# MikeIvanichev/norma

Hardware: AMD Instinct MI355X
Metric: audio-sec/wall-sec (xRT) distil-large-v3 fp16 b32 (higher is better)
Workload: dtype f16

## Files before the change

norma_amd/csrc/k_gemm.hip:

```cpp
#include <stdlib.h>

#include <atomic>

#include "mfma_tile128.h"

#define BM 128
#define BN 128
#define BK 64

__device__ __forceinline__ float gelu_tanh_f(float v) { return gelu_tanh_fast(v); }

__device__ __forceinline__ const half_t *a_row_ptr(const GemmParams &p, int m) {
    if (m >= p.M) m = p.M - 1;
    int b = nh_div(m, p.a_rpb, p.a_magic), r = m - b * p.a_rpb;
    return p.A + (long)b * p.a_bstride + (long)r * p.lda;
}

template <bool SWAP>
__device__ __forceinline__ void gemm_mainloop(const GemmParams &p, char *smem, int m0, int n0, f32x4 (&acc)[4][4]) {
    tile128_mainloop<SWAP>([&](int row) { return a_row_ptr(p, m0 + row); },
                           [&](int row) { return p.W + (long)(n0 + row) * p.K; }, p.K / BK, smem, acc);
}

__device__ __forceinline__ long out_row(const GemmParams &p, int m) {
    int b = nh_div(m, p.o_rpb, p.o_magic), r = m - b * p.o_rpb;
    return (long)b * p.o_bstride + r + p.o_off;
}

__global__ __launch_bounds__(256, 2) void gemm_f16_kernel(GemmParams p) {
    __shared__ __attribute__((aligned(16))) char smem[T128_LDS];
    const int ntn = p.N / BN, ntm = (p.M + BM - 1) / BM;
    const int bid = xcd_contiguous(blockIdx.x, ntn * ntm);
    const int tm = bid / ntn, tn = bid - tm * ntn;
    const int m0 = tm * BM, n0 = tn * BN;
    const int lane = threadIdx.x & 63, w = threadIdx.x >> 6;
    const int wm = w >> 1, wn = w & 1;
    const int fr = lane & 15, fq = lane >> 4;

    f32x4 acc[4][4];
#pragma unroll
    for (int i = 0; i < 4; i++)
#pragma unroll
        for (int j = 0; j < 4; j++) acc[i][j] = (f32x4){0.f, 0.f, 0.f, 0.f};

    const int seg = (p.epi == EPI_F16 || p.epi == EPI_GELU_F16) ? n0 / p.seg_n : 0;
    const bool vt = (p.epi == EPI_F16 && seg == p.vt_seg);
    if (vt) gemm_mainloop<false>(p, smem, m0, n0, acc);
    else gemm_mainloop<true>(p, smem, m0, n0, acc);

    if (vt) {
        half_t *dst = reinterpret_cast<half_t *>(seg == 0 ? p.out[0] : seg == 1 ? p.out[1] : p.out[2]);
#pragma unroll
        for (int i = 0; i < 4; i++) {
            int n = n0 + wn * 64 + 16 * i + fr;
            float bv = p.bias ? p.bias[n] : 0.f;
            int nl = n - seg * p.seg_n, h = nl >> 6, dh = nl & 63;
#pragma unroll
            for (int j = 0; j < 4; j++) {
                int m = m0 + wm * 64 + 16 * j + 4 * fq;
                if (m >= p.M) continue;
                int b = nh_div(m, p.S, p.s_magic), s = m - b * p.S;
                half_t *row = dst + ((long)(b * p.H + h) * NH_DH + dh) * NH_SP;
                if (s + 3 < p.S && m + 3 < p.M) {
                    half4 v = {(half_t)(acc[i][j][0] + bv), (half_t)(acc[i][j][1] + bv),
                               (half_t)(acc[i][j][2] + bv), (half_t)(acc[i][j][3] + bv)};
                    *reinterpret_cast<half4 *>(row + s) = v;
                } else {
                    for (int r = 0; r < 4; r++) {
                        int mm = m + r;
                        if (mm >= p.M) break;
                        int bb = nh_div(mm, p.S, p.s_magic), ss = mm - bb * p.S;
                        dst[((long)(bb * p.H + h) * NH_DH + dh) * NH_SP + ss] = (half_t)(acc[i][j][r] + bv);
                    }
                }
            }
        }
        return;
    }
    half_t *obase = reinterpret_cast<half_t *>(seg == 0 ? p.out[0] : seg == 1 ? p.out[1] : p.out[2]);
#pragma unroll
    for (int i = 0; i < 4; i++) {
        const int n = n0 + wn * 64 + 16 * i + 4 * fq;
        f32x4 bv = {0.f, 0.f, 0.f, 0.f};
        if (p.bias) bv = *reinterpret_cast<const f32x4 *>(p.bias + n);
#pragma unroll
        for (int j = 0; j < 4; j++) {
            const int m = m0 + wm * 64 + 16 * j + fr;
            if (m >= p.M) continue;
            f32x4 v = acc[i][j] + bv;
            if (p.epi == EPI_F16 || p.epi == EPI_GELU_F16) {
                if (p.epi == EPI_F16 && seg == 0 && p.seg0_scale != 0.f) v *= p.seg0_scale;
                if (p.epi == EPI_GELU_F16) {
                    v[0] = gelu_tanh_f(v[0]); v[1] = gelu_tanh_f(v[1]);
                    v[2] = gelu_tanh_f(v[2]); v[3] = gelu_tanh_f(v[3]);
                }
                const int nl = n - seg * p.seg_n;
                half_t *dst = p.head_major ? obase + (((long)nh_div(m, p.S, p.s_magic) * p.H + (nl >> 6)) * p.S + (m - nh_div(m, p.S, p.s_magic) * p.S)) * NH_DH + (nl & 63)
                                           : obase + out_row(p, m) * p.ldo + nl;
                half4 hv = {(half_t)v[0], (half_t)v[1], (half_t)v[2], (half_t)v[3]};
                *reinterpret_cast<half4 *>(dst) = hv;
            } else if (p.epi == EPI_RESID_F32) {
                float *dst = reinterpret_cast<float *>(p.out[0]) + (long)m * p.ldo + n;
                f32x4 x = *reinterpret_cast<const f32x4 *>(dst);
                *reinterpret_cast<f32x4 *>(dst) = x + v;
            } else {
                int s = m - nh_div(m, p.S, p.s_magic) * p.S;
                f32x4 pe = *reinterpret_cast<const f32x4 *>(p.pos + (long)s * p.N + n);
                f32x4 o = {gelu_tanh_f(v[0]) + pe[0], gelu_tanh_f(v[1]) + pe[1], gelu_tanh_f(v[2]) + pe[2],
                           gelu_tanh_f(v[3]) + pe[3]};
                *reinterpret_cast<f32x4 *>(reinterpret_cast<float *>(p.out[0]) + (long)m * p.ldo + n) = o;
            }
        }
    }
}

#define G2_BM 256
#define G2_BN 256
#define G2_GM 4
#define PP_BUF 65536
#define PP_HT 16384
#define PP_RING (2 * PP_BUF)
#define PP_EPI_PITCH 136
#define PP_EPI_WAVE (16 * PP_EPI_PITCH)

struct PPSource { unsigned ag[2][2], wg[2][2]; };

__device__ __forceinline__ PPSource pp_source(const GemmParams &p, int m0, int n0) {
    int tid = threadIdx.x;
    asm volatile("" : "+v"(tid));
    const int lrow = tid >> 3;
    const int csrc = ((tid & 7) ^ ((lrow >> 1) & 7)) * 8;
    PPSource sg;
#pragma unroll
    for (int h = 0; h < 2; h++)
#pragma unroll
        for (int i = 0; i < 2; i++) {
            sg.ag[h][i] = (unsigned)(a_row_ptr(p, m0 + i * 128 + h * 64 + lrow) - p.A) + csrc;
            const int l = lrow + 64 * i;
            sg.wg[h][i] = (unsigned)(n0 + (l >> 5) * 64 + h * 32 + (l & 31)) * (unsigned)p.K + csrc;
        }
    return sg;
}

__device__ __forceinline__ void pp_stage(const GemmParams &p, char *wbase, const PPSource &sg, int t, int which) {
    const int h = (which >> 1) & 1;
    const bool isB = which == 1 || which == 2;
    char *dst = wbase + (t & 1) * PP_BUF + (isB ? 2 * PP_HT : 0) + h * PP_HT;
    const unsigned ko = (unsigned)t * 64u;
    if (isB) {
        __builtin_amdgcn_global_load_lds((gbl_void *)(p.W + (size_t)(sg.wg[h][0] + ko)), (lds_void *)dst, 16, 0, 0);
        __builtin_amdgcn_global_load_lds((gbl_void *)(p.W + (size_t)(sg.wg[h][1] + ko)), (lds_void *)(dst + 8192), 16, 0, 0);
    } else {
        __builtin_amdgcn_global_load_lds((gbl_void *)(p.A + (size_t)(sg.ag[h][0] + ko)), (lds_void *)dst, 16, 0, 0);
        __builtin_amdgcn_global_load_lds((gbl_void *)(p.A + (size_t)(sg.ag[h][1] + ko)), (lds_void *)(dst + 8192), 16, 0, 0);
    }
}

__device__ __forceinline__ void pp_prologue(const GemmParams &p, char *wbase, const PPSource &sg) {
    pp_stage(p, wbase, sg, 0, 0); pp_stage(p, wbase, sg, 0, 1); pp_stage(p, wbase, sg, 0, 2); pp_stage(p, wbase, sg, 0, 3);
    pp_stage(p, wbase, sg, 1, 0); pp_stage(p, wbase, sg, 1, 1);
}

template <bool SWAP>
__device__ __forceinline__ void pp_main(const GemmParams &p, char *smem, char *wbase, const PPSource &sg, f32x4 (&acc)[8][4]) {
    const int lane = threadIdx.x & 63, w = threadIdx.x >> 6;
    const int wr = w >> 2, wc = w & 3;
    const int fr = lane & 15, fq = lane >> 4;
    const int nt = p.K >> 6;
    const int offA0 = (wr * 64 + fr) * 128 + ((fq ^ (fr >> 1)) << 4);
    const int offB0 = (wc * 32 + fr) * 128 + ((fq ^ (fr >> 1)) << 4);
    const char *const pa[2] = {smem + offA0, smem + (offA0 ^ 64)};
    const char *const pb[2] = {smem + offB0, smem + (offB0 ^ 64)};
    half8 fa[4][2], fb[4][2];

#define PP_PHASE(Q, BUF, WAIT, DO_ISSUE, ST)                                                                             \
    {                                                                                                                    \
        constexpr int tb_ = (BUF) * PP_BUF;                                                                              \
        if ((Q) == 0) {                                                                                                  \
            _Pragma("unroll") for (int j = 0; j < 2; j++) _Pragma("unroll") for (int ks = 0; ks < 2; ks++)             \
                fb[j][ks] = *reinterpret_cast<const half8 *>(pb[ks] + (tb_ + 2 * PP_HT + 2048 * j));                    \
            __builtin_amdgcn_sched_barrier(0);                                                                           \
            _Pragma("unroll") for (int i = 0; i < 4; i++) _Pragma("unroll") for (int ks = 0; ks < 2; ks++)             \
                fa[i][ks] = *reinterpret_cast<const half8 *>(pa[ks] + (tb_ + 2048 * i));                               \
        } else if ((Q) == 1) {                                                                                           \
            _Pragma("unroll") for (int j = 0; j < 2; j++) _Pragma("unroll") for (int ks = 0; ks < 2; ks++)             \
                fb[2 + j][ks] = *reinterpret_cast<const half8 *>(pb[ks] + (tb_ + 3 * PP_HT + 2048 * j));                \
        } else if ((Q) == 2) {                                                                                           \
            _Pragma("unroll") for (int i = 0; i < 4; i++) _Pragma("unroll") for (int ks = 0; ks < 2; ks++)             \
                fa[i][ks] = *reinterpret_cast<const half8 *>(pa[ks] + (tb_ + PP_HT + 2048 * i));                       \
        }                                                                                                                \
        __builtin_amdgcn_sched_barrier(0);                                                                               \
        if (DO_ISSUE) pp_stage(p, wbase, sg, (ST), (Q) == 2 ? 0 : (Q) == 3 ? 1 : (Q) == 0 ? 2 : 3);                     \
        if ((WAIT) == 8) asm volatile("s_waitcnt vmcnt(8)" ::: "memory");                                                \
        else if ((WAIT) == 4) asm volatile("s_waitcnt vmcnt(4)" ::: "memory");                                           \
        else if ((WAIT) == 2) asm volatile("s_waitcnt vmcnt(2)" ::: "memory");                                           \
        else if ((WAIT) == 0) asm volatile("s_waitcnt vmcnt(0)" ::: "memory");                                           \
        __builtin_amdgcn_s_barrier();                                                                                    \
        asm volatile("s_waitcnt lgkmcnt(0)" ::: "memory");                                                               \
        __builtin_amdgcn_sched_barrier(0);                                                                               \
        __builtin_amdgcn_s_setprio(1);                                                                                   \
        {                                                                                                                \
            constexpr int ib_ = ((Q) >= 2) ? 4 : 0, jb_ = ((Q) == 1 || (Q) == 2) ? 2 : 0;                                \
            _Pragma("unroll") for (int ks = 0; ks < 2; ks++) _Pragma("unroll") for (int i = 0; i < 4; i++)             \
                _Pragma("unroll") for (int j = 0; j < 2; j++) {                                                         \
                    if (SWAP) acc[ib_ + i][jb_ + j] = __builtin_amdgcn_mfma_f32_16x16x32_f16(fb[jb_ + j][ks], fa[i][ks], acc[ib_ + i][jb_ + j], 0, 0, 0); \
                    else acc[ib_ + i][jb_ + j] = __builtin_amdgcn_mfma_f32_16x16x32_f16(fa[i][ks], fb[jb_ + j][ks], acc[ib_ + i][jb_ + j], 0, 0, 0);      \
                }                                                                                                        \
        }                                                                                                                \
        __builtin_amdgcn_s_setprio(0);                                                                                   \
        __builtin_amdgcn_sched_barrier(0);                                                                               \
        __builtin_amdgcn_s_barrier();                                                                                    \
    }

    asm volatile("s_waitcnt vmcnt(0)" ::: "memory");
    __builtin_amdgcn_s_barrier();
    if (wr == 1) __builtin_amdgcn_s_barrier();
    int t = 0;
    for (; t + 4 <= nt; t += 2) {
        PP_PHASE(0, 0, 8, true, t + 1)
        PP_PHASE(1, 0, 8, true, t + 1)
        PP_PHASE(2, 0, -1, true, t + 2)
        PP_PHASE(3, 0, 8, true, t + 2)
        PP_PHASE(0, 1, 8, true, t + 2)
        PP_PHASE(1, 1, 8, true, t + 2)
        PP_PHASE(2, 1, -1, true, t + 3)
        PP_PHASE(3, 1, 8, true, t + 3)
    }
    PP_PHASE(0, 0, 8, true, t + 1)
    PP_PHASE(1, 0, 8, true, t + 1)
    PP_PHASE(2, 0, -1, false, 0)
    PP_PHASE(3, 0, 4, false, 0)
    PP_PHASE(0, 1, 2, false, 0)
    PP_PHASE(1, 1, 0, false, 0)
    PP_PHASE(2, 1, -1, false, 0)
    PP_PHASE(3, 1, -1, false, 0)
    if (wr == 0) __builtin_amdgcn_s_barrier();
#undef PP_PHASE
}

__device__ __forceinline__ void pp_tile(int vb, int ntn, int ntm, int &tm, int &tn) {
    grouped_tile(xcd_contiguous(vb, ntn * ntm), ntn, ntm, G2_GM, tm, tn);
}

template <int EPI>
__global__ __launch_bounds__(512) void gemm256_f16_kernel(GemmParams p) {
    __shared__ __attribute__((aligned(16))) char smem[PP_RING + 8 * PP_EPI_WAVE];
    const int ntn = p.N / G2_BN, ntm = (p.M + G2_BM - 1) / G2_BM, nwg = ntn * ntm;
    const int lane = threadIdx.x & 63, w = threadIdx.x >> 6;
    const int wm = w >> 2, wn = w & 3;
    const int fr = lane & 15, fq = lane >> 4;
    char *const wbase = smem + __builtin_amdgcn_readfirstlane(w) * 1024;
    char *const img = smem + PP_RING + w * PP_EPI_WAVE;

    int vb = blockIdx.x, tm, tn;
    pp_tile(vb, ntn, ntm, tm, tn);
    PPSource sg = pp_source(p, tm * G2_BM, tn * G2_BN);
    pp_prologue(p, wbase, sg);
    for (;;) {
        const int m0 = tm * G2_BM, n0 = tn * G2_BN;
        f32x4 acc[8][4];
#pragma unroll
        for (int i = 0; i < 8; i++)
#pragma unroll
            for (int j = 0; j < 4; j++) acc[i][j] = (f32x4){0.f, 0.f, 0.f, 0.f};
        const int seg = (EPI == EPI_F16 || EPI == EPI_GELU_F16) ? n0 / p.seg_n : 0;
        const bool vt = (EPI == EPI_F16 && seg == p.vt_seg);
        if (vt) pp_main<false>(p, smem, wbase, sg, acc);
        else pp_main<true>(p, smem, wbase, sg, acc);

        f32x4 rs[4][4];
        __amdgpu_buffer_rsrc_t xrs;
        unsigned xoff = 0;
        if (EPI == EPI_RESID_F32) {
            xrs = __builtin_amdgcn_make_buffer_rsrc(p.out[0], 0, (int)((long)p.M * p.ldo * 4), 0x00020000);
            int ln = threadIdx.x;
            asm volatile("" : "+v"(ln));
            xoff = (unsigned)(((long)(m0 + (ln >> 8) * 128 + (ln & 15)) * p.ldo + n0 + ((ln >> 6) & 3) * 64 + 4 * ((ln >> 4) & 3)) * 4);
#pragma unroll
            for (int ii = 0; ii < 4; ii++)
#pragma unroll
                for (int j = 0; j < 4; j++)
                    rs[ii][j] = __builtin_bit_cast(f32x4, __builtin_amdgcn_raw_buffer_load_b128(xrs, xoff + (unsigned)(64 * ii * p.ldo + 64 * j), 0, 0));
        }
        const int nvb = vb + gridDim.x;
        const bool more = nvb < nwg;
        if (more) {
            pp_tile(nvb, ntn, ntm, tm, tn);
            sg = pp_source(p, tm * G2_BM, tn * G2_BN);
            pp_prologue(p, wbase, sg);
        }

        if (vt) {
            half_t *dst = reinterpret_cast<half_t *>(seg == 0 ? p.out[0] : seg == 1 ? p.out[1] : p.out[2]);
#pragma unroll
            for (int j = 0; j < 4; j++) {
                const float bv = p.bias ? p.bias[n0 + wn * 64 + 16 * j + fr] : 0.f;
#pragma unroll
                for (int hh = 0; hh < 2; hh++) {
#pragma unroll
                    for (int ii = 0; ii < 4; ii++) {
                        const f32x4 a = acc[4 * hh + ii][j];
                        half4 v = {(half_t)(a[0] + bv), (half_t)(a[1] + bv), (half_t)(a[2] + bv), (half_t)(a[3] + bv)};
                        *reinterpret_cast<half4 *>(img + fr * PP_EPI_PITCH + (16 * ii + 4 * fq) * 2) = v;
                    }
#pragma unroll
                    for (int it = 0; it < 2; it++) {
                        const int nrow = 8 * it + (lane >> 3), mc = (lane & 7) * 8;
                        const half4 lo = *reinterpret_cast<const half4 *>(img + nrow * PP_EPI_PITCH + mc * 2);
                        const half4 hi = *reinterpret_cast<const half4 *>(img + nrow * PP_EPI_PITCH + mc * 2 + 8);
                        const int n = n0 + wn * 64 + 16 * j + nrow, nl = n - seg * p.seg_n, h = nl >> 6, dh = nl & 63;
                        const int m = m0 + wm * 128 + 64 * hh + mc;
                        if (m >= p.M) continue;
                        const int b = nh_div(m, p.S, p.s_magic), ss = m - b * p.S;
                        if (ss + 7 < p.S && m + 7 < p.M) {
                            half8 o = {lo[0], lo[1], lo[2], lo[3], hi[0], hi[1], hi[2], hi[3]};
                            *reinterpret_cast<half8 *>(dst + ((long)(b * p.H + h) * NH_DH + dh) * NH_SP + ss) = o;
                        } else {
                            for (int r = 0; r < 8; r++) {
                                const int mm = m + r;
                                if (mm >= p.M) break;
                                const int bb = nh_div(mm, p.S, p.s_magic), s2 = mm - bb * p.S;
                                dst[((long)(bb * p.H + h) * NH_DH + dh) * NH_SP + s2] = r < 4 ? lo[r] : hi[r - 4];
                            }
                        }
                    }
                }
            }
        } else if (EPI == EPI_F16 || EPI == EPI_GELU_F16) {
            half_t *ob = reinterpret_cast<half_t *>(seg == 0 ? p.out[0] : seg == 1 ? p.out[1] : p.out[2]);
            f32x4 bv[4];
#pragma unroll
            for (int j = 0; j < 4; j++) {
                bv[j] = (f32x4){0.f, 0.f, 0.f, 0.f};
                if (p.bias) bv[j] = *reinterpret_cast<const f32x4 *>(p.bias + n0 + wn * 64 + 16 * j + 4 * fq);
            }
            const int ncol = n0 + wn * 64 - seg * p.seg_n + (lane & 7) * 8;
            const bool q_scaled = EPI == EPI_F16 && seg == 0 && p.seg0_scale != 0.f;
#pragma unroll
            for (int i = 0; i < 8; i++) {
#pragma unroll
                for (int j = 0; j < 4; j++) {
                    f32x4 v = acc[i][j] + bv[j];
                    if (EPI == EPI_F16 && q_scaled) v *= p.seg0_scale;
                    if (EPI == EPI_GELU_F16) {
                        v[0] = gelu_tanh_f(v[0]); v[1] = gelu_tanh_f(v[1]); v[2] = gelu_tanh_f(v[2]); v[3] = gelu_tanh_f(v[3]);
                    }
                    half4 hv = {(half_t)v[0], (half_t)v[1], (half_t)v[2], (half_t)v[3]};
                    *reinterpret_cast<half4 *>(img + fr * PP_EPI_PITCH + (16 * j + 4 * fq) * 2) = hv;
                }
#pragma unroll
                for (int it = 0; it < 2; it++) {
                    const int mr = 8 * it + (lane >> 3);
                    const int m = m0 + wm * 128 + 16 * i + mr;
                    const half4 lo = *reinterpret_cast<const half4 *>(img + mr * PP_EPI_PITCH + (lane & 7) * 16);
                    const half4 hi = *reinterpret_cast<const half4 *>(img + mr * PP_EPI_PITCH + (lane & 7) * 16 + 8);
                    if (m < p.M) {
                        half8 o = {lo[0], lo[1], lo[2], lo[3], hi[0], hi[1], hi[2], hi[3]};
                        half_t *dst = p.head_major ? ob + (((long)nh_div(m, p.S, p.s_magic) * p.H + (ncol >> 6)) * p.S + (m - nh_div(m, p.S, p.s_magic) * p.S)) * NH_DH + (lane & 7) * 8
                                                   : ob + out_row(p, m) * p.ldo + ncol;
                        *reinterpret_cast<half8 *>(dst) = o;
                    }
                }
            }
        } else if (EPI == EPI_RESID_F32) {
            f32x4 bv[4];
#pragma unroll
            for (int j = 0; j < 4; j++) {
                bv[j] = (f32x4){0.f, 0.f, 0.f, 0.f};
                if (p.bias) bv[j] = *reinterpret_cast<const f32x4 *>(p.bias + n0 + wn * 64 + 16 * j + 4 * fq);
            }
#pragma unroll
            for (int ii = 0; ii < 4; ii++)
#pragma unroll
                for (int j = 0; j < 4; j++)
                    __builtin_amdgcn_raw_buffer_store_b128(__builtin_bit_cast(u32x4, rs[ii][j] + (acc[ii][j] + bv[j])), xrs, xoff + (unsigned)(64 * ii * p.ldo + 64 * j), 0, 0);
#pragma unroll
            for (int ii = 0; ii < 4; ii++)
#pragma unroll
                for (int j = 0; j < 4; j++)
                    rs[ii][j] = __builtin_bit_cast(f32x4, __builtin_amdgcn_raw_buffer_load_b128(xrs, xoff + (unsigned)(64 * (4 + ii) * p.ldo + 64 * j), 0, 0));
#pragma unroll
            for (int ii = 0; ii < 4; ii++)
#pragma unroll
                for (int j = 0; j < 4; j++)
                    __builtin_amdgcn_raw_buffer_store_b128(__builtin_bit_cast(u32x4, rs[ii][j] + (acc[4 + ii][j] + bv[j])), xrs, xoff + (unsigned)(64 * (4 + ii) * p.ldo + 64 * j), 0, 0);
        } else {
#pragma unroll
            for (int j = 0; j < 4; j++) {
                const int n = n0 + wn * 64 + 16 * j + 4 * fq;
                f32x4 bv = {0.f, 0.f, 0.f, 0.f};
                if (p.bias) bv = *reinterpret_cast<const f32x4 *>(p.bias + n);
#pragma unroll
                for (int i = 0; i < 8; i++) {
                    const int m = m0 + wm * 128 + 16 * i + fr;
                    if (m >= p.M) continue;
                    const f32x4 v = acc[i][j] + bv;
                    const int s = m - nh_div(m, p.S, p.s_magic) * p.S;
                    const f32x4 pe = *reinterpret_cast<const f32x4 *>(p.pos + (long)s * p.N + n);
                    f32x4 o = {gelu_tanh_f(v[0]) + pe[0], gelu_tanh_f(v[1]) + pe[1], gelu_tanh_f(v[2]) + pe[2],
                               gelu_tanh_f(v[3]) + pe[3]};
                    *reinterpret_cast<f32x4 *>(reinterpret_cast<float *>(p.out[0]) + (long)m * p.ldo + n) = o;
                }
            }
        }
        if (!more) break;
        vb = nvb;
    }
}

static int device_cu_count() {
    static std::atomic<int> cus[NH_MAX_DEVICES];
    int dev = 0;
    if (hipGetDevice(&dev) != hipSuccess || dev < 0 || dev >= NH_MAX_DEVICES) return 256;
    int n = cus[dev].load(std::memory_order_relaxed);
    if (!n) {
        if (hipDeviceGetAttribute(&n, hipDeviceAttributeMultiprocessorCount, dev) != hipSuccess || n <= 0) n = 256;
        cus[dev].store(n, std::memory_order_relaxed);
    }
    return n;
}

static GemmParams with_magics(const GemmParams &p_in) {
    GemmParams p = p_in;
    const long max_m = (long)p.M - 1;
    p.a_magic = nh_magic(p.a_rpb, max_m); p.o_magic = nh_magic(p.o_rpb, max_m); p.s_magic = nh_magic(p.S, max_m);
    return p;
}

void launch_gemm(const GemmParams &p_in, hipStream_t st) {
    const GemmParams p = with_magics(p_in);
    const bool seg_ok = (p.epi != EPI_F16 && p.epi != EPI_GELU_F16) || (p.seg_n % G2_BN == 0);
    if (p.N % G2_BN == 0 && p.K % 128 == 0 && seg_ok && p.M >= G2_BM) {
        const int nwg = (p.N / G2_BN) * ((p.M + G2_BM - 1) / G2_BM);
        int cus = p.cus > 0 ? p.cus : device_cu_count();
        cus -= cus % 8;
        const dim3 grid(nwg < cus ? nwg : cus), block(512);
        switch (p.epi) {
            case EPI_F16: hipLaunchKernelGGL(gemm256_f16_kernel<EPI_F16>, grid, block, 0, st, p); break;
            case EPI_GELU_F16: hipLaunchKernelGGL(gemm256_f16_kernel<EPI_GELU_F16>, grid, block, 0, st, p); break;
            case EPI_RESID_F32: hipLaunchKernelGGL(gemm256_f16_kernel<EPI_RESID_F32>, grid, block, 0, st, p); break;
            default: hipLaunchKernelGGL(gemm256_f16_kernel<EPI_CONV2_F32>, grid, block, 0, st, p); break;
        }
        return;
    }
    launch_gemm_128(p, st);
}

void launch_gemm_128(const GemmParams &p_in, hipStream_t st) {
    const GemmParams p = with_magics(p_in);
    int ntn = p.N / BN, ntm = (p.M + BM - 1) / BM;
    hipLaunchKernelGGL(gemm_f16_kernel, dim3(ntn * ntm), dim3(256), 0, st, p);
}
```

norma_amd/csrc/nh_kernels.h:

```cpp
#pragma once
#include <hip/hip_runtime.h>
#include <math.h>
#include <stdint.h>

#include <atomic>

#include "skinny_plan.h"

typedef _Float16 half_t;
typedef __attribute__((ext_vector_type(8))) _Float16 half8;
typedef __attribute__((ext_vector_type(4))) _Float16 half4;
typedef __attribute__((ext_vector_type(2))) _Float16 half2v;
typedef __attribute__((ext_vector_type(2))) float f32x2;
typedef __attribute__((ext_vector_type(4))) float f32x4;
typedef __attribute__((ext_vector_type(16))) float f32x16;
typedef __attribute__((ext_vector_type(4))) unsigned int u32x4;

#define NH_MELP 128
#define NH_SP 1536
#define NH_DH 64
#define NH_MAX_DEVICES 64
#define NH_MAX_VOCAB 65536

enum GemmEpi {
    EPI_F16 = 0,
    EPI_GELU_F16 = 1,
    EPI_RESID_F32 = 2,
    EPI_CONV2_F32 = 3,
};

struct GemmParams {
    const half_t *A; long lda; int a_rpb; long a_bstride;
    const half_t *W;
    const float *bias;
    int M, N, K;
    int epi;
    void *out[3]; int seg_n; long ldo;
    int o_rpb; long o_bstride; long o_off;
    int vt_seg;
    int head_major;
    float seg0_scale;
    int S, H;
    const float *pos;
    int cus;
    unsigned a_magic, o_magic, s_magic;
};
static inline unsigned nh_magic(int d, long max_m) {
    if (d <= 0 || (long)d > max_m) return 0u;
    if ((unsigned long long)max_m * (unsigned long long)d >= 0x100000000ull) return ~0u;
    return (unsigned)((0x100000000ull + (unsigned)d - 1) / (unsigned)d);
}
#ifdef __HIPCC__
__device__ __forceinline__ int nh_div(int m, int d, unsigned magic) {
    return magic == 0u ? 0 : magic == ~0u ? m / d : (int)__umulhi((unsigned)m, magic);
}
#endif
void launch_gemm(const GemmParams &p, hipStream_t st);
void launch_gemm_128(const GemmParams &p, hipStream_t st);

struct SkinnyParams {
    const half_t *x; long ldx;
    const half_t *W; const float *bias;
    const half_t *Wt;
    int R, N, K;
    int epi;
    void *out[3]; long ldo;
    int d, t0, Tn, ctx;
    const int32_t *pos_ptr;
    const float *ln_x, *ln_w, *ln_b;
    float ln_rk;
};
inline bool skinny_ln_supported(int R, int N, int K) { return skinny_plan(R, N, K, SK_F32, false, true).kind != SKP_NONE; }

#ifdef __HIPCC__
__device__ __forceinline__ float gelu_tanh_fast(float v) {
#pragma clang fp contract(off)
    const float k0 = -2.0f * 0.7978845608028654f * 1.4426950408889634f;
    const float k1 = k0 * 0.044715f;
    const float m = v * __builtin_fmaf(v * v, k1, k0);
    float r = v * __builtin_amdgcn_rcpf(1.0f + __builtin_amdgcn_exp2f(m));
    asm("" : "+v"(r));
    return r;
}
__device__ __forceinline__ float ln_sum8(float acc, const f32x4 &a, const f32x4 &b) {
#pragma clang fp contract(off)
    acc += (a[0] + a[1]) + (a[2] + a[3]);
    acc += (b[0] + b[1]) + (b[2] + b[3]);
    return acc;
}
__device__ __forceinline__ float ln_sq8(float acc, const f32x4 &a, const f32x4 &b, float mean) {
#pragma clang fp contract(off)
    const f32x4 t = a - mean, u = b - mean;
    acc += __builtin_fmaf(t[1], t[1], t[0] * t[0]) + __builtin_fmaf(t[3], t[3], t[2] * t[2]);
    acc += __builtin_fmaf(u[1], u[1], u[0] * u[0]) + __builtin_fmaf(u[3], u[3], u[2] * u[2]);
    return acc;
}
__device__ __forceinline__ float ln_mean(float sum, float rk) {
#pragma clang fp contract(off)
    return sum * rk;
}
__device__ __forceinline__ float ln_inv(float sumsq, float rk) {
#pragma clang fp contract(off)
    const float var = sumsq * rk;
    return 1.0f / sqrtf(var + 1e-5f);
}
__device__ __forceinline__ f32x4 ln_apply(const f32x4 &x, float mean, float inv, const f32x4 &g, const f32x4 &b) {
#pragma clang fp contract(off)
    const f32x4 t = (x - mean) * inv;
    f32x4 o = {__builtin_fmaf(t[0], g[0], b[0]), __builtin_fmaf(t[1], g[1], b[1]), __builtin_fmaf(t[2], g[2], b[2]),
               __builtin_fmaf(t[3], g[3], b[3])};
    asm("" : "+v"(o));
    return o;
}
#endif
bool launch_layernorm_sliced(const float *x, const float *w, const float *b, half_t *y, float *y32, int M, int K, hipStream_t st);
[[nodiscard]] bool launch_skinny(const SkinnyParams &p, hipStream_t st);
void launch_repack_tiles(const half_t *W, half_t *out, int N, int K, hipStream_t st);

#define NH_LDS_EXCLUSIVE (160 * 1024)
#ifdef __HIPCC__
static inline size_t lds_exclusive_bytes(size_t needed) {
#ifdef NH_DBG_SHARE_LDS
    return needed;
#else
    (void)needed;
    return (size_t)NH_LDS_EXCLUSIVE;
#endif
}
template <auto Kernel, class... Args>
static void launch_lds_exclusive(dim3 grid, dim3 block, size_t lds_used, hipStream_t st, Args... args) {
    static std::atomic<bool> attr_set[NH_MAX_DEVICES];
    int dev = 0;
    (void)hipGetDevice(&dev);
    if (dev < 0 || dev >= NH_MAX_DEVICES || !attr_set[dev].load(std::memory_order_acquire)) {
        hipFuncSetAttribute(reinterpret_cast<const void *>(Kernel), hipFuncAttributeMaxDynamicSharedMemorySize, NH_LDS_EXCLUSIVE);
        if (dev >= 0 && dev < NH_MAX_DEVICES) attr_set[dev].store(true, std::memory_order_release);
    }
    hipLaunchKernelGGL(Kernel, grid, block, lds_exclusive_bytes(lds_used), st, args...);
}
#endif

void launch_layernorm(const float *x, const float *w, const float *b, half_t *y, float *y32, int M, int d,
                      hipStream_t st);
void launch_embed(const int32_t *tokens, int tok_stride, const half_t *E, const half_t *P, float *x, int B,
                  int Tn, int t0, const int32_t *pos_ptr, int d, hipStream_t st);

#ifdef __HIPCC__
template <typename T> __device__ __forceinline__ float sample_to_f32(T v);
template <> __device__ __forceinline__ float sample_to_f32<float>(float v) { return v; }
template <> __device__ __forceinline__ float sample_to_f32<double>(double v) { return (float)v; }
template <> __device__ __forceinline__ float sample_to_f32<int8_t>(int8_t v) { return (float)v * (1.0f / 128.0f); }
template <> __device__ __forceinline__ float sample_to_f32<int16_t>(int16_t v) { return (float)v * (1.0f / 32768.0f); }
template <> __device__ __forceinline__ float sample_to_f32<int32_t>(int32_t v) { return (float)v * (1.0f / 2147483648.0f); }
template <> __device__ __forceinline__ float sample_to_f32<int64_t>(int64_t v) { return (float)v * (1.0f / 9223372036854775808.0f); }
template <> __device__ __forceinline__ float sample_to_f32<uint8_t>(uint8_t v) { return (float)((int)v - 128) * (1.0f / 128.0f); }
template <> __device__ __forceinline__ float sample_to_f32<uint16_t>(uint16_t v) { return (float)((int)v - 32768) * (1.0f / 32768.0f); }
template <> __device__ __forceinline__ float sample_to_f32<uint32_t>(uint32_t v) { return (float)(int32_t)(v ^ 0x80000000u) * (1.0f / 2147483648.0f); }
template <> __device__ __forceinline__ float sample_to_f32<uint64_t>(uint64_t v) { return (float)(int64_t)(v ^ 0x8000000000000000ull) * (1.0f / 9223372036854775808.0f); }
#endif

struct ResampleClip {
    long long off;
    long long num0;
    int n_frames;
    int n_out;
};
struct ResampleParams {
    const void *frames;
    int dtype, channels;
    const ResampleClip *clips; int batch;
    const float *coef;
    int L, M, T;
    float *out; long out_stride;
    int max_out;
};
#define NH_RS_TILE 2048
static inline size_t resample_lds_bytes(int L, int M, int T) {
    return sizeof(float) * (size_t)(((long long)(NH_RS_TILE - 1) * M + L - 1) / L + T + 2);
}
[[nodiscard]] bool launch_resample(const ResampleParams &p, hipStream_t st);

#define NH_CUT_FRAME 160
#define NH_CUT_TILE 128
#define NH_CUT_ROW 161
static inline size_t cut_lds_bytes() { return sizeof(float) * (size_t)NH_CUT_TILE * NH_CUT_ROW; }
void launch_cut_energy(const float *pcm, long long n_valid, float *e, long long n_frames, hipStream_t st);
void launch_cut_window(const float *e, float *E, long long F, int W, hipStream_t st);
struct CutSearch {
    const float *E; long long F;
    int min_frames, max_frames;
    long long n_samples;
    long long *starts; int32_t *lens;
    int32_t *count;
    long long cap;
};
void launch_cut_search(const CutSearch &p, hipStream_t st);
#ifdef __HIPCC__
__device__ __forceinline__ void cut_merge(float &best, int &c, float ob, int oc) {
    if (oc >= 0 && (c < 0 || ob < best || (ob == best && oc > c))) { best = ob; c = oc; }
}
__device__ __forceinline__ int cut_search_range(const float *E, long long s, int min_frames, int max_frames, float *w_best, int *w_c) {
    const int tid = threadIdx.x;
    float best = INFINITY;
    int c = -1;
    for (int r = min_frames + tid; r <= max_frames; r += 256) {
        const float v = E[s + r];
        if (v <= best) { best = v; c = r; }
    }
#pragma unroll
    for (int off = 32; off > 0; off >>= 1) {
        const float ob = __shfl_xor(best, off);
        const int oc = __shfl_xor(c, off);
        cut_merge(best, c, ob, oc);
    }
    if ((tid & 63) == 0) { w_best[tid >> 6] = best; w_c[tid >> 6] = c; }
    __syncthreads();
    best = w_best[0]; c = w_c[0];
    for (int w = 1; w < 4; w++) cut_merge(best, c, w_best[w], w_c[w]);
    __syncthreads();
    return c < 0 ? max_frames : c;
}
#endif

#define NH_VAD_HIST_TILE 4096
#define NH_VAD_TILE 2048
struct VadSelect {
    unsigned hist[2][256];
    unsigned prefix[2];
    long long rank[2];
    int parted;
    int n_valid;
};
struct VadLevels {
    int lo_permille, hi_permille;
    float lo_ratio, hi_ratio, abs_floor;
};
void launch_vad_hist(const float *E, long long F, int shift, VadSelect *sel, hipStream_t st);
void launch_vad_pick(VadSelect *sel, int shift, const VadLevels &lv, float *levels, hipStream_t st);
struct VadShape {
    const float *E; const float *levels;
    long long F;
    const uint8_t *in; uint8_t *out;
    const int *carry_l, *carry_r;
    int *tile_l, *tile_r;
    int min_speech, pad, min_gap;
    long long *regions; const int *carry_n;
};
void launch_vad_shape(int step, const VadShape &p, hipStream_t st);
void launch_vad_carry(const int *tile_l, const int *tile_r, int *carry_l, int *carry_r, int n_tiles, long long F, int sum, int *total, hipStream_t st);
struct VadPieces {
    const float *E; const long long *regions; const int *n_regions;
    int min_frames, max_frames;
    long long n_samples;
    long long *starts; int32_t *lens; long long cap_pieces;
    int32_t *chunk_first; long long cap_chunks;
    int32_t *counts;
};
void launch_vad_pieces(const VadPieces &p, hipStream_t st);
struct VadGather {
    const float *src; float *dst; long long dst_stride;
    const long long *tab;
    int n_pieces, vec4;
};
void launch_vad_gather(const VadGather &p, int batch, long long max_total, hipStream_t st);

struct MelTables {
    const float *hann;
    const float *dft_cos;
    const float *dft_sin;
    const float *tw_cos;
    const float *tw_sin;
    const float *filters;
};
void launch_logmel_grp(const float *pcm, const int32_t *n_samples, long stride, const MelTables &t,
                       const int32_t *grp, int n_mel, int frames, float *mel32, unsigned *chunk_max, int B,
                       hipStream_t st);
void launch_mel_finish_ex(float *mel32, const unsigned *chunk_max, half_t *img, int B, int n_mel, int frames,
                          int normalise, hipStream_t st);

#define NH_ENC_Q_SCALE (0.125f * 1.4426950408889634f)
void launch_enc_attention(const half_t *q, const half_t *k, long ld, const half_t *vt, half_t *out, long ldo,
                          int B, int S, int H, hipStream_t st);

void launch_dec_attention(const half_t *q, const half_t *kc, const half_t *vc, half_t *out, int B, int H, int d, int ctx, int Tk,
                          const int32_t *pos_ptr, hipStream_t st, const int32_t *done);

bool launch_prefill_self_attention(const half_t *q, const half_t *k, const half_t *v, long ld, half_t *out, long ldo, half_t *ck,
                                   half_t *cv, int B, int T, int H, int C, hipStream_t st);
bool launch_prefill_cross_attention(const half_t *q, long ldq, const half_t *ck, const half_t *cv, half_t *out, long ldo, int B, int T,
                                    int H, int S, hipStream_t st);

void launch_xabs_attention(const half_t *q, const half_t *Wkv, const float *bkv, const half_t *xa, half_t *U, half_t *out, int B, int H, int d, int S,
                           const int32_t *done, hipStream_t st);

bool xabs_fast_supported(int d, int H);
void launch_transpose_sq(const half_t *in, half_t *out, int d, hipStream_t st);
void launch_xabs_attention_fast(const half_t *q, const half_t *WkT, const half_t *Wkv, const float *bkv, const half_t *xa, half_t *U, float *zpart, float *mlpart,
                                half_t *out, int B, int H, int d, int S, const int32_t *done, hipStream_t st);

struct DecodeState {
    int32_t *tokens;
    int32_t *n_tokens;
    int32_t *done;
    int32_t *have_last;
    int32_t *last_ts;
    double *sum_logprob;
    double *no_speech;
    int32_t *n_active;
    const uint8_t *suppress;
};
struct RuleTokens { int sot, eot, lang, task, no_speech, no_timestamps, zero_sec, one_sec; };
inline int nh_logits_ld(int V) { return (V + 63) & ~63; }
void launch_logit_step(const float *logits, int V, DecodeState s, RuleTokens tk, int B, int ctx, int cap,
                       int max_new, int prompt_len, int mode, float *partials, unsigned *tickets, int32_t *pos_ptr,
                       hipStream_t st, const int32_t *handled = nullptr);
void launch_pool_admit(DecodeState s, int32_t *pos, unsigned *tickets, int row, int ctx, int t0, int t1, int t2, int P, hipStream_t st,
                       int32_t *detect_flag = nullptr, int detect = 0);
struct PoolSampling {
    float *inv_t;
    unsigned long long *seed;
    unsigned *clip, *attempt;
    int32_t *handled;
};
void launch_pool_retry(DecodeState s, int32_t *pos, unsigned *tickets, PoolSampling ps, int row, int P, float inv_t,
                       unsigned long long seed, unsigned clip, unsigned attempt, hipStream_t st, int32_t *detect_flag = nullptr);
void launch_pool_sample_step(const float *logits, int V, DecodeState s, RuleTokens tk, int B, int ctx, int cap, int max_new,
                             int prompt_len, PoolSampling ps, int32_t *pos, hipStream_t st);
void launch_sample_step(const float *logits, int V, DecodeState s, RuleTokens tk, int B, int ctx, int cap, int max_new,
                        int prompt_len, float inv_t, unsigned long long seed, unsigned clip0, unsigned attempt, hipStream_t st);
void launch_sample_rules(const float *probs_in, int32_t *token_out, const int32_t *tokens, int n_tokens, int last_ts,
                         const uint8_t *suppress, RuleTokens tk, int V, float inv_t, unsigned long long seed, unsigned clip,
                         unsigned attempt, hipStream_t st);
void launch_lang_detect(const float *logits, int V, const int32_t *lang_tokens, int n, float *probs_out, int32_t *lang_out,
                        int B, hipStream_t st);
struct PoolDetect {
    const int32_t *flag;
    const int32_t *lang_tokens;
    int n;
    int32_t *lang_out;
    float *probs;
};
void launch_pool_lang_detect(const float *logits, int V, DecodeState s, int B, int ctx, const int32_t *pos, PoolDetect det,
                             hipStream_t st);
#define NH_GUARD_MAX_BIAS 256
#define NH_GUARD_MAX_PERIOD 64
#define NH_GUARD_MAX_HISTORY 512
struct GuardSpec { int ngram; float penalty; int loop_period, loop_repeats, bias; };
struct GuardBufs {
    const int32_t *bias_tok;
    const float *bias_val;
    const int32_t *bias_n;
    const int32_t *bias_map;
    int bias_mod;
    int32_t *loop_exit;
};
void launch_guard(float *logits, int V, DecodeState s, RuleTokens tk, int R, int ctx, int prompt_len, const int32_t *pos, GuardSpec g,
                  GuardBufs gb, hipStream_t st);
void launch_rules_only(const float *probs_in, float *masked_out, int32_t *argmax_out, const int32_t *tokens,
                       int n_tokens, int last_ts, const uint8_t *suppress, RuleTokens tk, int V, hipStream_t st);

#define NH_ALIGN_HEADS 32
struct AlignLayerHeads { int32_t slot[NH_ALIGN_HEADS], head[NH_ALIGN_HEADS]; int n; };
void launch_align_qsave(const half_t *dq, half_t *q, const AlignLayerHeads &lh, int B, int ldb, int d, int pos, const int32_t *pos_ptr,
                        const int32_t *done, int npos, hipStream_t st);
struct AlignHeadPtrs { const half_t *q[NH_ALIGN_HEADS]; const half_t *k[NH_ALIGN_HEADS]; };
bool launch_align_weights(const AlignHeadPtrs &hp, int A, long q_pos_stride, long q_clip_stride, long k_clip_stride, const int32_t *n_rows,
                          const int32_t *n_keys, int max_rows, int S, int nclips, int clip0, float *W, long w_clip_stride, long w_head_stride,
                          long ldw, const int32_t *row_map, hipStream_t st);
bool launch_align_reduce(const float *W, long w_clip_stride, long w_head_stride, long ldw, const int32_t *n_rows, const int32_t *n_keys,
                         int max_rows, int S, int nclips, int clip0, int A, int P, float *stats, float *M, long m_clip_stride, long ldm,
                         const int32_t *row_map, hipStream_t st);
bool launch_align_dtw(const float *M, long m_clip_stride, long ldm, const int32_t *n_rows, const int32_t *n_keys, int P, int max_rows, int S,
                      int nclips, int clip0, uint8_t *trace, long t_clip_stride, int32_t *first, int32_t *last, int ldo, const int32_t *row_map,
                      hipStream_t st);

#ifndef NH_MAX_BEAMS
#define NH_MAX_BEAMS 8
#endif
struct BeamBufs {
    int32_t *parent;
    int32_t *fin_tokens;
    int32_t *fin_n;
    double *fin_score;
    int32_t *fin_count;
};
void launch_beam_select(const float *logits, int V, DecodeState s, RuleTokens tk, int R, int ctx, int K1, int32_t *cand_tok,
                        float *cand_q, int32_t *cand_n, hipStream_t st);
void launch_beam_merge(DecodeState s, RuleTokens tk, int V, int B, int K, int ctx, int cap, int max_new, int prompt_len,
                       const int32_t *cand_tok, const float *cand_q, const int32_t *cand_n, BeamBufs bb, hipStream_t st);
void launch_beam_reorder(half_t *const *caches, int n_caches, const int32_t *parent, int B, int K, int H, int C, int npos,
                         hipStream_t st);

int score_panel_rows(int V);
bool launch_score_rows(const half_t *xn, int M, int d, const half_t *E, int V, const int32_t *target, float *part, float *tlogit,
                       int T, long ldo, int off, float *out, int panel_rows, hipStream_t st);
```

Before: 6792.

## Stage bias via async LDS loads and precompute 32-bit epilogue store offsets

```diff
diff --git a/norma_amd/csrc/k_gemm.hip b/norma_amd/csrc/k_gemm.hip
--- a/norma_amd/csrc/k_gemm.hip
+++ b/norma_amd/csrc/k_gemm.hip
@@ -122,6 +122,9 @@
 #define PP_RING (2 * PP_BUF)
 #define PP_EPI_PITCH 136
 #define PP_EPI_WAVE (16 * PP_EPI_PITCH)
+#define PP_BIAS (PP_RING + 8 * PP_EPI_WAVE)
+#define PP_LDS (PP_BIAS + 2 * 1024)
+#define PP_VT_OOB 0xf0000000u
 
 struct PPSource { unsigned ag[2][2], wg[2][2]; };
 
@@ -135,7 +138,8 @@
     for (int h = 0; h < 2; h++)
 #pragma unroll
         for (int i = 0; i < 2; i++) {
-            sg.ag[h][i] = (unsigned)(a_row_ptr(p, m0 + i * 128 + h * 64 + lrow) - p.A) + csrc;
+            const unsigned m = (unsigned)min(m0 + i * 128 + h * 64 + lrow, p.M - 1), b = __umulhi(m, p.a_magic);
+            sg.ag[h][i] = b * (unsigned)p.a_bstride + (m - b * (unsigned)p.a_rpb) * (unsigned)p.lda + csrc;
             const int l = lrow + 64 * i;
             sg.wg[h][i] = (unsigned)(n0 + (l >> 5) * 64 + h * 32 + (l & 31)) * (unsigned)p.K + csrc;
         }
@@ -242,31 +246,186 @@
     grouped_tile(xcd_contiguous(vb, ntn * ntm), ntn, ntm, G2_GM, tm, tn);
 }
 
+
+__device__ __forceinline__ void pp_bias_stage(const GemmParams &p, char *smem, int w, int n0, int par) {
+    if (!p.bias) return;
+    int ln = threadIdx.x;
+    asm volatile("" : "+v"(ln));
+    __builtin_amdgcn_global_load_lds((gbl_void *)(p.bias + n0 + (w & 3) * 64 + (ln & 63)), (lds_void *)(smem + PP_BIAS + par * 1024 + (w & 3) * 256), 4, 0, 0);
+}
+
+__device__ __forceinline__ bool pp_next(const GemmParams &p, char *smem, int w, int par, int &vb, int ntn, int ntm, int &tm, int &tn, PPSource &sg) {
+    const int nvb = vb + gridDim.x;
+    if (nvb >= ntn * ntm) return false;
+    vb = nvb;
+    pp_tile(nvb, ntn, ntm, tm, tn);
+    pp_bias_stage(p, smem, w, tn * G2_BN, par ^ 1);
+    sg = pp_source(p, tm * G2_BM, tn * G2_BN);
+    pp_prologue(p, smem + w * 1024, sg);
+    return true;
+}
+
+__device__ __forceinline__ void pp_row_offsets(const GemmParams &p, int m0, int wm, int ln, unsigned (&off)[16]) {
+    const unsigned ml = (unsigned)(m0 + wm * 128 + ((ln >> 3) & 7)), lc = (unsigned)(ln & 7) * 16u;
+    const unsigned b0 = __umulhi((unsigned)m0, p.e_magic);
+    if (m0 + G2_BM <= p.M && b0 == __umulhi((unsigned)m0 + G2_BM - 1, p.e_magic)) {
+        const unsigned base = (b0 * p.e_db + ml) * p.e_rs + lc;
+#pragma unroll
+        for (int k = 0; k < 16; k++) off[k] = base + (unsigned)(8 * k) * p.e_rs;
+    } else {
+#pragma unroll
+        for (int k = 0; k < 16; k++) {
+            const unsigned m = ml + 8 * k;
+            off[k] = (__umulhi(m, p.e_magic) * p.e_db + m) * p.e_rs + lc;
+        }
+    }
+}
+
+__device__ __forceinline__ void pp_bias4(const char *smem, int par, int wn, int ln, f32x4 (&bv)[4]) {
+    const char *const src = smem + PP_BIAS + par * 1024 + wn * 256 + ((ln >> 4) & 3) * 16;
+#pragma unroll
+    for (int j = 0; j < 4; j++) bv[j] = *reinterpret_cast<const f32x4 *>(src + 64 * j);
+}
+
+template <bool GELU, bool SCALED>
+__device__ __forceinline__ void pp_epi_f16(const f32x4 (&acc)[8][4], const f32x4 (&bv)[4], float scale, char *img, int ln,
+                                           __amdgpu_buffer_rsrc_t ors, const unsigned (&off)[16]) {
+    char *const wr = img + (ln & 15) * PP_EPI_PITCH + ((ln >> 4) & 3) * 8;
+    const char *const rd = img + ((ln >> 3) & 7) * PP_EPI_PITCH + (ln & 7) * 16;
+#pragma unroll
+    for (int i = 0; i < 8; i++) {
+#pragma unroll
+        for (int j = 0; j < 4; j++) {
+            f32x4 v = acc[i][j] + bv[j];
+            if (SCALED) v *= scale;
+            if (GELU) {
+                v[0] = gelu_tanh_f(v[0]); v[1] = gelu_tanh_f(v[1]); v[2] = gelu_tanh_f(v[2]); v[3] = gelu_tanh_f(v[3]);
+            }
+            half4 hv = {(half_t)v[0], (half_t)v[1], (half_t)v[2], (half_t)v[3]};
+            *reinterpret_cast<half4 *>(wr + 32 * j) = hv;
+        }
+#pragma unroll
+        for (int it = 0; it < 2; it++) {
+            const half4 lo = *reinterpret_cast<const half4 *>(rd + 8 * it * PP_EPI_PITCH);
+            const half4 hi = *reinterpret_cast<const half4 *>(rd + 8 * it * PP_EPI_PITCH + 8);
+            const half8 o = {lo[0], lo[1], lo[2], lo[3], hi[0], hi[1], hi[2], hi[3]};
+            __builtin_amdgcn_raw_buffer_store_b128(__builtin_bit_cast(u32x4, o), ors, off[2 * i + it], 0, 0);
+        }
+    }
+}
+
+__device__ __forceinline__ void pp_epi_vt(const GemmParams &p, const f32x4 (&acc)[8][4], const float (&bv)[4], char *img, int ln,
+                                          half_t *dst, int m0, int wm, int nl0, bool one_clip, unsigned b0) {
+    char *const wr = img + (ln & 15) * PP_EPI_PITCH + ((ln >> 4) & 3) * 8;
+    const char *const rd = img + ((ln >> 3) & 7) * PP_EPI_PITCH + (ln & 7) * 16;
+    const int nl = nl0 + ((ln >> 3) & 7), ml = m0 + wm * 128 + (ln & 7) * 8;
+    __amdgpu_buffer_rsrc_t vrs = __builtin_amdgcn_make_buffer_rsrc(dst, 0, (int)p.vt_bytes, 0x00020000);
+    const unsigned voff = ((b0 * (unsigned)(p.H * NH_DH) + (unsigned)nl) * NH_SP + ((unsigned)ml - b0 * (unsigned)p.S)) * 2u;
+    bool whole[2];
+    unsigned wo[2];
+    if (!one_clip) {
+#pragma unroll
+        for (int hh = 0; hh < 2; hh++) {
+            const int m = ml + 64 * hh;
+            const unsigned b = __umulhi((unsigned)m, p.s_magic), ss = (unsigned)m - b * (unsigned)p.S;
+            whole[hh] = (int)ss + 7 < p.S && m + 7 < p.M;
+            wo[hh] = ((b * (unsigned)(p.H * NH_DH) + (unsigned)nl) * NH_SP + ss) * 2u;
+        }
+    }
+#pragma unroll
+    for (int j = 0; j < 4; j++) {
+#pragma unroll
+        for (int hh = 0; hh < 2; hh++) {
+#pragma unroll
+            for (int ii = 0; ii < 4; ii++) {
+                const f32x4 a = acc[4 * hh + ii][j];
+                half4 v = {(half_t)(a[0] + bv[j]), (half_t)(a[1] + bv[j]), (half_t)(a[2] + bv[j]), (half_t)(a[3] + bv[j])};
+                *reinterpret_cast<half4 *>(wr + 32 * ii) = v;
+            }
+#pragma unroll
+            for (int it = 0; it < 2; it++) {
+                const half4 lo = *reinterpret_cast<const half4 *>(rd + 8 * it * PP_EPI_PITCH);
+                const half4 hi = *reinterpret_cast<const half4 *>(rd + 8 * it * PP_EPI_PITCH + 8);
+                if (one_clip) {
+                    const half8 o = {lo[0], lo[1], lo[2], lo[3], hi[0], hi[1], hi[2], hi[3]};
+                    __builtin_amdgcn_raw_buffer_store_b128(__builtin_bit_cast(u32x4, o), vrs, voff + (unsigned)(((16 * j + 8 * it) * NH_SP + 64 * hh) * 2), 0, 0);
+                } else {
+                    const unsigned c = (unsigned)((16 * j + 8 * it) * NH_SP * 2);
+                    if (whole[hh]) {
+                        const half8 o = {lo[0], lo[1], lo[2], lo[3], hi[0], hi[1], hi[2], hi[3]};
+                        __builtin_amdgcn_raw_buffer_store_b128(__builtin_bit_cast(u32x4, o), vrs, wo[hh] + c, 0, 0);
+                    } else {
+#pragma unroll
+                        for (int r = 0; r < 8; r++) {
+                            const unsigned mm = (unsigned)(ml + 64 * hh + r), bb = __umulhi(mm, p.s_magic);
+                            const unsigned eo = (int)mm < p.M ? ((bb * (unsigned)(p.H * NH_DH) + (unsigned)nl) * NH_SP + (mm - bb * (unsigned)p.S)) * 2u : PP_VT_OOB;
+                            __builtin_amdgcn_raw_buffer_store_b16(__builtin_bit_cast(short, r < 4 ? lo[r] : hi[r - 4]), vrs, eo + c, 0, 0);
+                        }
+                    }
+                }
+            }
+        }
+    }
+}
+
 template <int EPI>
 __global__ __launch_bounds__(512) void gemm256_f16_kernel(GemmParams p) {
-    __shared__ __attribute__((aligned(16))) char smem[PP_RING + 8 * PP_EPI_WAVE];
-    const int ntn = p.N / G2_BN, ntm = (p.M + G2_BM - 1) / G2_BM, nwg = ntn * ntm;
-    const int lane = threadIdx.x & 63, w = threadIdx.x >> 6;
+    __shared__ __attribute__((aligned(16))) char smem[PP_LDS];
+    const int ntn = p.N / G2_BN, ntm = (p.M + G2_BM - 1) / G2_BM;
+    const int lane = threadIdx.x & 63, w = __builtin_amdgcn_readfirstlane(threadIdx.x >> 6);
     const int wm = w >> 2, wn = w & 3;
     const int fr = lane & 15, fq = lane >> 4;
-    char *const wbase = smem + __builtin_amdgcn_readfirstlane(w) * 1024;
+    char *const wbase = smem + w * 1024;
     char *const img = smem + PP_RING + w * PP_EPI_WAVE;
 
     int vb = blockIdx.x, tm, tn;
     pp_tile(vb, ntn, ntm, tm, tn);
+    if (!p.bias) *reinterpret_cast<float *>(smem + PP_BIAS + threadIdx.x * 4) = 0.f;
+    pp_bias_stage(p, smem, w, tn * G2_BN, 0);
     PPSource sg = pp_source(p, tm * G2_BM, tn * G2_BN);
     pp_prologue(p, wbase, sg);
-    for (;;) {
+    for (int par = 0;; par ^= 1) {
         const int m0 = tm * G2_BM, n0 = tn * G2_BN;
         f32x4 acc[8][4];
 #pragma unroll
         for (int i = 0; i < 8; i++)
 #pragma unroll
             for (int j = 0; j < 4; j++) acc[i][j] = (f32x4){0.f, 0.f, 0.f, 0.f};
-        const int seg = (EPI == EPI_F16 || EPI == EPI_GELU_F16) ? n0 / p.seg_n : 0;
-        const bool vt = (EPI == EPI_F16 && seg == p.vt_seg);
-        if (vt) pp_main<false>(p, smem, wbase, sg, acc);
-        else pp_main<true>(p, smem, wbase, sg, acc);
+        if (EPI == EPI_F16 || EPI == EPI_GELU_F16) {
+            const int stn = p.seg_n / G2_BN, seg = (tn >= stn) + (tn >= 2 * stn);
+            half_t *const ob = reinterpret_cast<half_t *>(seg == 0 ? p.out[0] : seg == 1 ? p.out[1] : p.out[2]);
+            const int nl0 = n0 - seg * p.seg_n + wn * 64;
+            if (EPI == EPI_F16 && seg == p.vt_seg) {
+                pp_main<false>(p, smem, wbase, sg, acc);
+                int ln = threadIdx.x;
+                asm volatile("" : "+v"(ln));
+                const unsigned b0 = __umulhi((unsigned)m0, p.s_magic);
+                const bool one_clip = m0 + G2_BM <= p.M && b0 == __umulhi((unsigned)m0 + G2_BM - 1, p.s_magic);
+                const bool more = pp_next(p, smem, w, par, vb, ntn, ntm, tm, tn, sg);
+                asm volatile("" : "+v"(ln));
+                float bv[4];
+#pragma unroll
+                for (int j = 0; j < 4; j++) bv[j] = *reinterpret_cast<const float *>(smem + PP_BIAS + par * 1024 + wn * 256 + 64 * j + (ln & 15) * 4);
+                pp_epi_vt(p, acc, bv, img, ln, ob, m0, wm, nl0, one_clip, b0);
+                if (!more) break;
+            } else {
+                pp_main<true>(p, smem, wbase, sg, acc);
+                int ln = threadIdx.x;
+                asm volatile("" : "+v"(ln));
+                f32x4 bv[4];
+                pp_bias4(smem, par, wn, ln, bv);
+                const __amdgpu_buffer_rsrc_t ors = __builtin_amdgcn_make_buffer_rsrc(reinterpret_cast<char *>(ob) + p.e_off0 + (long)nl0 * p.e_cs, 0, (int)p.e_bound, 0x00020000);
+                unsigned off[16];
+                pp_row_offsets(p, m0, wm, ln, off);
+                const bool more = pp_next(p, smem, w, par, vb, ntn, ntm, tm, tn, sg);
+                if (EPI == EPI_GELU_F16) pp_epi_f16<true, false>(acc, bv, 0.f, img, ln, ors, off);
+                else if (seg == 0 && p.seg0_scale != 0.f) pp_epi_f16<false, true>(acc, bv, p.seg0_scale, img, ln, ors, off);
+                else pp_epi_f16<false, false>(acc, bv, 0.f, img, ln, ors, off);
+                if (!more) break;
+            }
+            continue;
+        }
+        pp_main<true>(p, smem, wbase, sg, acc);
 
         f32x4 rs[4][4];
         __amdgpu_buffer_rsrc_t xrs;
@@ -282,93 +441,11 @@
                 for (int j = 0; j < 4; j++)
                     rs[ii][j] = __builtin_bit_cast(f32x4, __builtin_amdgcn_raw_buffer_load_b128(xrs, xoff + (unsigned)(64 * ii * p.ldo + 64 * j), 0, 0));
         }
-        const int nvb = vb + gridDim.x;
-        const bool more = nvb < nwg;
-        if (more) {
-            pp_tile(nvb, ntn, ntm, tm, tn);
-            sg = pp_source(p, tm * G2_BM, tn * G2_BN);
-            pp_prologue(p, wbase, sg);
-        }
-
-        if (vt) {
-            half_t *dst = reinterpret_cast<half_t *>(seg == 0 ? p.out[0] : seg == 1 ? p.out[1] : p.out[2]);
-#pragma unroll
-            for (int j = 0; j < 4; j++) {
-                const float bv = p.bias ? p.bias[n0 + wn * 64 + 16 * j + fr] : 0.f;
-#pragma unroll
-                for (int hh = 0; hh < 2; hh++) {
-#pragma unroll
-                    for (int ii = 0; ii < 4; ii++) {
-                        const f32x4 a = acc[4 * hh + ii][j];
-                        half4 v = {(half_t)(a[0] + bv), (half_t)(a[1] + bv), (half_t)(a[2] + bv), (half_t)(a[3] + bv)};
-                        *reinterpret_cast<half4 *>(img + fr * PP_EPI_PITCH + (16 * ii + 4 * fq) * 2) = v;
-                    }
-#pragma unroll
-                    for (int it = 0; it < 2; it++) {
-                        const int nrow = 8 * it + (lane >> 3), mc = (lane & 7) * 8;
-                        const half4 lo = *reinterpret_cast<const half4 *>(img + nrow * PP_EPI_PITCH + mc * 2);
-                        const half4 hi = *reinterpret_cast<const half4 *>(img + nrow * PP_EPI_PITCH + mc * 2 + 8);
-                        const int n = n0 + wn * 64 + 16 * j + nrow, nl = n - seg * p.seg_n, h = nl >> 6, dh = nl & 63;
-                        const int m = m0 + wm * 128 + 64 * hh + mc;
-                        if (m >= p.M) continue;
-                        const int b = nh_div(m, p.S, p.s_magic), ss = m - b * p.S;
-                        if (ss + 7 < p.S && m + 7 < p.M) {
-                            half8 o = {lo[0], lo[1], lo[2], lo[3], hi[0], hi[1], hi[2], hi[3]};
-                            *reinterpret_cast<half8 *>(dst + ((long)(b * p.H + h) * NH_DH + dh) * NH_SP + ss) = o;
-                        } else {
-                            for (int r = 0; r < 8; r++) {
-                                const int mm = m + r;
-                                if (mm >= p.M) break;
-                                const int bb = nh_div(mm, p.S, p.s_magic), s2 = mm - bb * p.S;
-                                dst[((long)(bb * p.H + h) * NH_DH + dh) * NH_SP + s2] = r < 4 ? lo[r] : hi[r - 4];
-                            }
-                        }
-                    }
-                }
-            }
-        } else if (EPI == EPI_F16 || EPI == EPI_GELU_F16) {
-            half_t *ob = reinterpret_cast<half_t *>(seg == 0 ? p.out[0] : seg == 1 ? p.out[1] : p.out[2]);
-            f32x4 bv[4];
-#pragma unroll
-            for (int j = 0; j < 4; j++) {
-                bv[j] = (f32x4){0.f, 0.f, 0.f, 0.f};
-                if (p.bias) bv[j] = *reinterpret_cast<const f32x4 *>(p.bias + n0 + wn * 64 + 16 * j + 4 * fq);
-            }
-            const int ncol = n0 + wn * 64 - seg * p.seg_n + (lane & 7) * 8;
-            const bool q_scaled = EPI == EPI_F16 && seg == 0 && p.seg0_scale != 0.f;
-#pragma unroll
-            for (int i = 0; i < 8; i++) {
-#pragma unroll
-                for (int j = 0; j < 4; j++) {
-                    f32x4 v = acc[i][j] + bv[j];
-                    if (EPI == EPI_F16 && q_scaled) v *= p.seg0_scale;
-                    if (EPI == EPI_GELU_F16) {
-                        v[0] = gelu_tanh_f(v[0]); v[1] = gelu_tanh_f(v[1]); v[2] = gelu_tanh_f(v[2]); v[3] = gelu_tanh_f(v[3]);
-                    }
-                    half4 hv = {(half_t)v[0], (half_t)v[1], (half_t)v[2], (half_t)v[3]};
-                    *reinterpret_cast<half4 *>(img + fr * PP_EPI_PITCH + (16 * j + 4 * fq) * 2) = hv;
-                }
-#pragma unroll
-                for (int it = 0; it < 2; it++) {
-                    const int mr = 8 * it + (lane >> 3);
-                    const int m = m0 + wm * 128 + 16 * i + mr;
-                    const half4 lo = *reinterpret_cast<const half4 *>(img + mr * PP_EPI_PITCH + (lane & 7) * 16);
-                    const half4 hi = *reinterpret_cast<const half4 *>(img + mr * PP_EPI_PITCH + (lane & 7) * 16 + 8);
-                    if (m < p.M) {
-                        half8 o = {lo[0], lo[1], lo[2], lo[3], hi[0], hi[1], hi[2], hi[3]};
-                        half_t *dst = p.head_major ? ob + (((long)nh_div(m, p.S, p.s_magic) * p.H + (ncol >> 6)) * p.S + (m - nh_div(m, p.S, p.s_magic) * p.S)) * NH_DH + (lane & 7) * 8
-                                                   : ob + out_row(p, m) * p.ldo + ncol;
-                        *reinterpret_cast<half8 *>(dst) = o;
-                    }
-                }
-            }
-        } else if (EPI == EPI_RESID_F32) {
-            f32x4 bv[4];
-#pragma unroll
-            for (int j = 0; j < 4; j++) {
-                bv[j] = (f32x4){0.f, 0.f, 0.f, 0.f};
-                if (p.bias) bv[j] = *reinterpret_cast<const f32x4 *>(p.bias + n0 + wn * 64 + 16 * j + 4 * fq);
-            }
+        const bool more = pp_next(p, smem, w, par, vb, ntn, ntm, tm, tn, sg);
+        f32x4 bv[4];
+        pp_bias4(smem, par, wn, lane, bv);
+
+        if (EPI == EPI_RESID_F32) {
 #pragma unroll
             for (int ii = 0; ii < 4; ii++)
 #pragma unroll
@@ -388,14 +465,12 @@
 #pragma unroll
             for (int j = 0; j < 4; j++) {
                 const int n = n0 + wn * 64 + 16 * j + 4 * fq;
-                f32x4 bv = {0.f, 0.f, 0.f, 0.f};
-                if (p.bias) bv = *reinterpret_cast<const f32x4 *>(p.bias + n);
 #pragma unroll
                 for (int i = 0; i < 8; i++) {
                     const int m = m0 + wm * 128 + 16 * i + fr;
                     if (m >= p.M) continue;
-                    const f32x4 v = acc[i][j] + bv;
-                    const int s = m - nh_div(m, p.S, p.s_magic) * p.S;
+                    const f32x4 v = acc[i][j] + bv[j];
+                    const int s = m - (int)__umulhi((unsigned)m, p.s_magic) * p.S;
                     const f32x4 pe = *reinterpret_cast<const f32x4 *>(p.pos + (long)s * p.N + n);
                     f32x4 o = {gelu_tanh_f(v[0]) + pe[0], gelu_tanh_f(v[1]) + pe[1], gelu_tanh_f(v[2]) + pe[2],
                                gelu_tanh_f(v[3]) + pe[3]};
@@ -404,7 +479,6 @@
             }
         }
         if (!more) break;
-        vb = nvb;
     }
 }
 
@@ -427,10 +501,42 @@
     return p;
 }
 
+static bool plan_gemm256(GemmParams &p) {
+    const bool f16 = p.epi == EPI_F16 || p.epi == EPI_GELU_F16;
+    if (p.N % G2_BN != 0 || p.K % 128 != 0 || p.M < G2_BM || (f16 && p.seg_n % G2_BN != 0)) return false;
+    const unsigned long long lim = 0xffffffffull;
+    const long rows = ((long)p.M + G2_BM - 1) / G2_BM * G2_BM;
+    if (p.a_magic == ~0u || p.s_magic == ~0u) return false;
+    if ((unsigned long long)(p.a_magic ? (p.M - 1) / p.a_rpb : 0) * p.a_bstride + (unsigned long long)p.M * p.lda + p.K > lim) return false;
+    if (p.s_magic != 0u) {
+        p.s_magic = nh_magic(p.S, rows - 1);
+        if (p.s_magic == ~0u) return false;
+    }
+    if (!f16) return true;
+    const bool hm = p.epi == EPI_F16 && p.head_major;
+    const long rpb = hm ? p.S : p.o_rpb, bstride = hm ? (long)p.H * p.S : p.o_bstride;
+    p.e_rs = hm ? NH_DH * 2 : (unsigned)(p.ldo * 2);
+    p.e_cs = hm ? 2L * p.S : 2L;
+    p.e_off0 = hm ? 0L : p.o_off * p.ldo * 2;
+    p.e_magic = (rpb <= 0 || rpb >= p.M) ? 0u : nh_magic((int)rpb, rows - 1);
+    if (p.e_magic == ~0u || (p.e_magic != 0u && bstride < rpb) || p.ldo * 2 > (long)lim || p.e_rs < 128u) return false;
+    p.e_db = p.e_magic ? (unsigned)(bstride - rpb) : 0u;
+    const unsigned long long last = ((unsigned long long)(p.e_magic ? (p.M - 1) / rpb : 0) * p.e_db + (unsigned long long)(p.M - 1)) * p.e_rs + 128;
+    const unsigned long long far = ((unsigned long long)(p.e_magic ? (rows - 1) / rpb : 0) * p.e_db + (unsigned long long)(rows - 1)) * p.e_rs + 128;
+    if (far > lim) return false;
+    p.e_bound = (unsigned)last;
+    if (p.epi == EPI_F16 && p.vt_seg >= 0) {
+        if (p.S <= 0) return false;
+        const unsigned long long vb = (unsigned long long)((p.M + p.S - 1) / p.S) * p.H * NH_DH * NH_SP * 2;
+        if (vb > PP_VT_OOB) return false;
+        p.vt_bytes = (unsigned)vb;
+    }
+    return true;
+}
+
 void launch_gemm(const GemmParams &p_in, hipStream_t st) {
-    const GemmParams p = with_magics(p_in);
-    const bool seg_ok = (p.epi != EPI_F16 && p.epi != EPI_GELU_F16) || (p.seg_n % G2_BN == 0);
-    if (p.N % G2_BN == 0 && p.K % 128 == 0 && seg_ok && p.M >= G2_BM) {
+    GemmParams p = with_magics(p_in);
+    if (plan_gemm256(p)) {
         const int nwg = (p.N / G2_BN) * ((p.M + G2_BM - 1) / G2_BM);
         int cus = p.cus > 0 ? p.cus : device_cu_count();
         cus -= cus % 8;
diff --git a/norma_amd/csrc/nh_kernels.h b/norma_amd/csrc/nh_kernels.h
--- a/norma_amd/csrc/nh_kernels.h
+++ b/norma_amd/csrc/nh_kernels.h
@@ -44,6 +44,8 @@
     const float *pos;
     int cus;
     unsigned a_magic, o_magic, s_magic;
+    unsigned e_magic, e_db, e_rs, e_bound, vt_bytes;
+    long e_off0, e_cs;
 };
 static inline unsigned nh_magic(int d, long max_m) {
     if (d <= 0 || (long)d > max_m) return 0u;
```

After: 6919, median of 6. +1.9%, better.
